# jyjblrd/Low-Cost-Mocap

Measured on NVIDIA H100. Metric: mocap frame-sets/s (4-cam 640x480 synthetic, blob+epipolar+DLT), higher is better.
Workload: dtype u8 pixels -> int64 moments -> f64 geometry

## Files before the change

low-cost-mocap_b200/csrc/fused_common.cuh:

```cuda
#pragma once
#include "common.cuh"
#include "blob_device.cuh"
#include "match_device.cuh"

struct FusedParams {
    const uint4* frames;
    long long total_units;
    int n_sets, C, W, H;
    int seg_per_image, units_per_image, iters_per_unit;
    int u4_per_image;
    int threshold;
    ThreshConst tc;
    int E;
    uint32_t* seg_count; uint32_t* seg_list;
    uint32_t* img_done;
    uint32_t* set_done;
    uint32_t* set_defer;
    unsigned long long* unit_counter;
    int32_t* blob_xy; int32_t* blob_n; int32_t* img_flags;
    uint32_t* img_worklist; uint32_t* img_work_count;
    uint32_t* set_worklist; uint32_t* set_work_count;
    const CameraTables* tb;
    int MB, RMAX, KC; uint32_t GMAX;
    double* obj; double* err; int32_t* n_obj; int32_t* set_flags;
    int32_t* track_xy;
    size_t slab_bytes;
};

template <bool WIDE>
__device__ __forceinline__ void finish_image(const FusedParams& P, unsigned char* slab, int img, int lane) {
    __threadfence();
    const unsigned cnt = __ldcg(&P.seg_count[img]);
    bool deferred = false;
    if (cnt == 0) {
        if (lane == 0) { P.blob_n[img] = 0; if (P.img_flags) P.img_flags[img] = 0; }
    } else {
        bool ok = cnt <= BLOB_WE;
        if (ok) {
            WarpSlab& sl = *reinterpret_cast<WarpSlab*>(slab);
            BlobSmem sm;
            sm.seg = sl.seg; sm.parent = sl.parent; sm.base = sl.base; sm.node_seg = sl.node_seg;
            sm.node_bits = sl.node_bits; sm.rank = sl.rank; sm.acc = sl.acc; sm.wsum = nullptr; sm.hs = nullptr;
    sm.rowfirst = BLOB_ROWFIRST(sl, WIDE); sm.row_cap = WIDE ? 0 : BLOB_ROWS;
            const uint32_t* lst = P.seg_list + (size_t)img * P.E;
            for (int i = lane; i < (int)cnt; i += 32) sm.seg[i] = __ldcg(lst + i);
            __syncwarp();
            ok = blob_reduce<32, true, WIDE>(sm, (int)cnt, BLOB_WE, BLOB_WACC, P.W, P.H, P.MB,
                                             P.blob_xy + (size_t)img * P.MB * 2, P.blob_n + img, nullptr,
                                             P.img_flags ? P.img_flags + img : nullptr, 0);
            __syncwarp();
        }
        if (lane == 0) {
            if (ok) P.seg_count[img] = 0;
            else P.img_worklist[atomicAdd(P.img_work_count, 1u)] = (uint32_t)img;
        }
        deferred = !ok;
    }
    if (lane == 0) { P.img_done[img] = 0; }
    const int set = img / P.C;
    if (deferred && lane == 0) atomicOr(&P.set_defer[set], 1u);
    __threadfence();
    __syncwarp();
    unsigned sd = 0;
    if (lane == 0) {
        __threadfence();
        sd = atomicAdd(&P.set_done[set], 1u);
    }
    sd = __shfl_sync(0xffffffffu, sd, 0);
    if (sd != (unsigned)P.C - 1) return;

    __threadfence();
    const unsigned defer = __ldcg(&P.set_defer[set]);
    __syncwarp();
    if (lane == 0) { P.set_done[set] = 0; P.set_defer[set] = 0; }
    if (defer) {
        if (lane == 0) P.set_worklist[atomicAdd(P.set_work_count, 1u)] = (uint32_t)set;
        return;
    }
    WarpState ws = carve_warp_state(slab, P.RMAX, P.C, P.KC, P.MB);
    match_triangulate_warp(P.tb, ws, P.blob_xy + (size_t)set * P.C * P.MB * 2, P.blob_n + (size_t)set * P.C, set, lane,
                           P.C, P.MB, P.RMAX, P.KC, P.GMAX, P.obj, P.err, P.n_obj, P.set_flags, nullptr, P.track_xy,
                           P.img_flags ? P.img_flags + (size_t)set * P.C : nullptr);
    __syncwarp();
}
```

low-cost-mocap_b200/csrc/fused_device.cuh:

```cuda
#pragma once
#include "fused_common.cuh"

#define FUSED_WARPS 8
#define FUSED_UNROLL 6
#define FUSED_SEGS_PER_ITER (32 * FUSED_UNROLL)

template <bool USE_AND, bool CH3>
__device__ __forceinline__ void fused_hit(const FusedParams& P, int img, const uint4* __restrict__ src, int si, const uint4& v) {
    uint32_t m, seg;
    if (!CH3) {
        const uint32_t h0 = swar_gt(v.x, P.tc), h1 = swar_gt(v.y, P.tc);
        const uint32_t h2 = swar_gt(v.z, P.tc), h3 = swar_gt(v.w, P.tc);
        m = nibble_of(h0) | (nibble_of(h1) << 4) | (nibble_of(h2) << 8) | (nibble_of(h3) << 12);
        seg = (uint32_t)si;
    } else {
        seg = (uint32_t)si / 3u;
        const int r = si - 3 * (int)seg;
        uint32_t w[12];
        bool earlier = false;
#pragma unroll
        for (int q = 0; q < 3; ++q) {
            const uint4 x = __ldg(src + 3 * seg + q);
            if (q < r && any_above<USE_AND>(x, P.tc)) earlier = true;
            w[4 * q + 0] = x.x; w[4 * q + 1] = x.y; w[4 * q + 2] = x.z; w[4 * q + 3] = x.w;
        }
        if (earlier) return;
        m = 0;
#pragma unroll
        for (int p = 0; p < 16; ++p) {
            const int o = 3 * p;
            const uint32_t c0 = (w[o >> 2] >> ((o & 3) * 8)) & 0xffu;
            const uint32_t c1 = (w[(o + 1) >> 2] >> (((o + 1) & 3) * 8)) & 0xffu;
            const uint32_t c2 = (w[(o + 2) >> 2] >> (((o + 2) & 3) * 8)) & 0xffu;
            const int grey = (int)((c0 * 9798u + c1 * 19235u + c2 * 3735u + 16384u) >> 15);
            m |= (grey > P.threshold ? 1u : 0u) << p;
        }
        if (!m) return;
    }
    const uint32_t slot = atomicAdd(&P.seg_count[img], 1u);
    if (slot < (uint32_t)P.E) P.seg_list[(size_t)img * P.E + slot] = (seg << 16) | m;
}

template <bool WIDE, bool USE_AND, bool CH3 = false>
__global__ void __launch_bounds__(FUSED_WARPS * 32, 4)
k_pipeline_fused(const FusedParams P) {
    extern __shared__ __align__(16) unsigned char smem_raw[];
    const int warp = threadIdx.x >> 5, lane = threadIdx.x & 31;
    unsigned char* slab = smem_raw + P.slab_bytes * warp;

    while (true) {
        unsigned long long u = 0;
        if (lane == 0) u = atomicAdd(P.unit_counter, 1ull);
        u = __shfl_sync(0xffffffffu, u, 0);
        if (u >= (unsigned long long)P.total_units) break;
        const int img = (int)(u / P.units_per_image);
        const int unit = (int)(u - (unsigned long long)img * P.units_per_image);

        const int s_begin = unit * P.iters_per_unit * FUSED_SEGS_PER_ITER;
        const int s_end = min(P.u4_per_image, s_begin + P.iters_per_unit * FUSED_SEGS_PER_ITER);
        const uint4* src = P.frames + (size_t)img * P.u4_per_image;
        const int n_full = (s_end - s_begin) / FUSED_SEGS_PER_ITER;
        if (n_full > 0) {
            const uint4* sp = src + s_begin + lane;
            uint4 v[FUSED_UNROLL];
#pragma unroll
            for (int q = 0; q < FUSED_UNROLL; ++q) v[q] = ldg_stream(sp + q * 32);
            for (int it = 0; it < n_full; ++it) {
                const bool more = it + 1 < n_full;
                const uint4* nx = sp + (it + 1) * FUSED_SEGS_PER_ITER;
#pragma unroll
                for (int q = 0; q < FUSED_UNROLL; ++q) {
                    if (any_above<USE_AND>(v[q], P.tc))
                        fused_hit<USE_AND, CH3>(P, img, src, s_begin + it * FUSED_SEGS_PER_ITER + q * 32 + lane, v[q]);
                    if (more) v[q] = ldg_stream(nx + q * 32);
                }
            }
        }
        for (int si = s_begin + n_full * FUSED_SEGS_PER_ITER + lane; si < s_end; si += 32) {
            const uint4 x = ldg_stream(src + si);
            if (any_above<USE_AND>(x, P.tc)) fused_hit<USE_AND, CH3>(P, img, src, si, x);
        }
        __threadfence();
        __syncwarp();
        unsigned done = 0;
        if (lane == 0) {
            __threadfence();
            done = atomicAdd(&P.img_done[img], 1u);
        }
        done = __shfl_sync(0xffffffffu, done, 0);
        if (done != (unsigned)P.units_per_image - 1) continue;

        finish_image<WIDE>(P, slab, img, lane);
    }
}
```

Measured before the change: 2.376 million.

## Interleave unit chunks across image and replace threadfences with acq_rel fences

Each work unit now reads strided 192-segment chunks interleaved across the image (unit, unit+U, ...) instead of a contiguous block, so warps working on the same image at the same time touch nearby addresses. The tail segments go to the last unit. Redundant double __threadfence calls are replaced by a single fence.acq_rel.gpu from lane 0 plus __syncwarp. The lighter fences risk weaker visibility of other lanes' seg_list writes if the cumulativity assumption does not hold.

```diff
diff --git a/low-cost-mocap_b200/csrc/fused_common.cuh b/low-cost-mocap_b200/csrc/fused_common.cuh
--- a/low-cost-mocap_b200/csrc/fused_common.cuh
+++ b/low-cost-mocap_b200/csrc/fused_common.cuh
@@ -27,9 +27,18 @@
     size_t slab_bytes;
 };
 
+__device__ __forceinline__ void fence_acq_rel_gpu() {
+#if defined(__CUDACC__)
+    asm volatile("fence.acq_rel.gpu;" ::: "memory");
+#else
+    __threadfence();
+#endif
+}
+
 template <bool WIDE>
 __device__ __forceinline__ void finish_image(const FusedParams& P, unsigned char* slab, int img, int lane) {
-    __threadfence();
+    fence_acq_rel_gpu();
+    __syncwarp();
     const unsigned cnt = __ldcg(&P.seg_count[img]);
     bool deferred = false;
     if (cnt == 0) {
@@ -59,17 +68,17 @@
     if (lane == 0) { P.img_done[img] = 0; }
     const int set = img / P.C;
     if (deferred && lane == 0) atomicOr(&P.set_defer[set], 1u);
-    __threadfence();
     __syncwarp();
     unsigned sd = 0;
     if (lane == 0) {
-        __threadfence();
+        fence_acq_rel_gpu();
         sd = atomicAdd(&P.set_done[set], 1u);
     }
     sd = __shfl_sync(0xffffffffu, sd, 0);
     if (sd != (unsigned)P.C - 1) return;
 
-    __threadfence();
+    fence_acq_rel_gpu();
+    __syncwarp();
     const unsigned defer = __ldcg(&P.set_defer[set]);
     __syncwarp();
     if (lane == 0) { P.set_done[set] = 0; P.set_defer[set] = 0; }
diff --git a/low-cost-mocap_b200/csrc/fused_device.cuh b/low-cost-mocap_b200/csrc/fused_device.cuh
--- a/low-cost-mocap_b200/csrc/fused_device.cuh
+++ b/low-cost-mocap_b200/csrc/fused_device.cuh
@@ -56,35 +56,37 @@
         const int img = (int)(u / P.units_per_image);
         const int unit = (int)(u - (unsigned long long)img * P.units_per_image);
 
-        const int s_begin = unit * P.iters_per_unit * FUSED_SEGS_PER_ITER;
-        const int s_end = min(P.u4_per_image, s_begin + P.iters_per_unit * FUSED_SEGS_PER_ITER);
+        const int U = P.units_per_image;
+        const int n_iter_img = P.u4_per_image / FUSED_SEGS_PER_ITER;
         const uint4* src = P.frames + (size_t)img * P.u4_per_image;
-        const int n_full = (s_end - s_begin) / FUSED_SEGS_PER_ITER;
+        const int n_full = unit < n_iter_img ? (n_iter_img - unit + U - 1) / U : 0;
         if (n_full > 0) {
-            const uint4* sp = src + s_begin + lane;
+            const uint4* sp = src + unit * FUSED_SEGS_PER_ITER + lane;
+            const int stride = U * FUSED_SEGS_PER_ITER;
             uint4 v[FUSED_UNROLL];
 #pragma unroll
             for (int q = 0; q < FUSED_UNROLL; ++q) v[q] = ldg_stream(sp + q * 32);
             for (int it = 0; it < n_full; ++it) {
                 const bool more = it + 1 < n_full;
-                const uint4* nx = sp + (it + 1) * FUSED_SEGS_PER_ITER;
+                const uint4* nx = sp + (it + 1) * stride;
+                const int s0 = (unit + it * U) * FUSED_SEGS_PER_ITER + lane;
 #pragma unroll
                 for (int q = 0; q < FUSED_UNROLL; ++q) {
                     if (any_above<USE_AND>(v[q], P.tc))
-                        fused_hit<USE_AND, CH3>(P, img, src, s_begin + it * FUSED_SEGS_PER_ITER + q * 32 + lane, v[q]);
+                        fused_hit<USE_AND, CH3>(P, img, src, s0 + q * 32, v[q]);
                     if (more) v[q] = ldg_stream(nx + q * 32);
                 }
             }
         }
-        for (int si = s_begin + n_full * FUSED_SEGS_PER_ITER + lane; si < s_end; si += 32) {
-            const uint4 x = ldg_stream(src + si);
-            if (any_above<USE_AND>(x, P.tc)) fused_hit<USE_AND, CH3>(P, img, src, si, x);
-        }
-        __threadfence();
+        if (unit == U - 1)
+            for (int si = n_iter_img * FUSED_SEGS_PER_ITER + lane; si < P.u4_per_image; si += 32) {
+                const uint4 x = ldg_stream(src + si);
+                if (any_above<USE_AND>(x, P.tc)) fused_hit<USE_AND, CH3>(P, img, src, si, x);
+            }
         __syncwarp();
         unsigned done = 0;
         if (lane == 0) {
-            __threadfence();
+            fence_acq_rel_gpu();
             done = atomicAdd(&P.img_done[img], 1u);
         }
         done = __shfl_sync(0xffffffffu, done, 0);
```

New measurement: 2.385 million, median of 6. No clear change (+0.4%).
